# cyh-0/CAVP

Hardware: AMD Instinct MI355X
Metric: frames/sec end-to-end CAVP fwd+bwd, B=32 224x224 (higher is better)
Workload: dtype bf16; 1 GPU; C1' (config_avss_binary shape): CAVP ResNet-50 OS16 + VGGish, training step = forward_train (batch-stat BN, 32 images + 64 audio clips per GPU) + cross-entropy + full backward, 224x224 RGB + 96x64 mel, num_classes=2, random-init (synthetic) weights; global_batch=32, per_gpu_batch=32, parallelism=dp1, ranks=1, launch=hipGraph replay, deterministic=False

## Files before the change

### cavp_amd/_lib.py

```python
from __future__ import annotations

import ctypes as C
import os

import torch

HERE = os.path.dirname(os.path.abspath(__file__))
LIB_PATH = os.path.join(HERE, "libcavp_hip.so")

F32, BF16, I64 = 0, 1, 2
ACT_NONE, ACT_RELU, ACT_LEAKY, ACT_GELU = 0, 1, 2, 3
ABI_VERSION = 16
ERR_BAD_ARG, ERR_UNSUPPORTED, ERR_ALIGN, ERR_WORKSPACE, ERR_LAUNCH = -1, -2, -3, -4, -5
WGRAD_GROUP_MAX = 16


class CavpError(RuntimeError):
    pass


class ConvDesc(C.Structure):
    _fields_ = [(n, C.c_int32) for n in (
        "dtype", "N", "H", "W", "Cin", "ldx", "Cout", "ldy", "KH", "KW", "stride", "pad", "dil", "ldr", "act",
        "splitk", "tile", "up", "Ho", "Wo", "stride_w", "dw_oihw", "dw_overwrite", "res_rows", "aux_mode", "ld_aux")]
# ... 67 lines not shown
    "cavp_grad_accumulate": (_i32, [_vp, _i32, _i32, _vp, _vp, _vp, _vp]),
    "cavp_accum_advance": (_i32, [_vp, _vp, _vp, _vp]),
    "cavp_optimizer_schedule_gated": (_i32, [_vp, _vp, _vp]),
    "cavp_optimizer_step_dev_gated": (_i32, [_vp, _i32, _i32, C.c_float, C.c_float, _vp, _vp, _vp]),
    "cavp_grad_guard_partials_gated": (_i32, [_vp, _i32, _i32, _vp, _vp, _vp]),
    "cavp_grad_guard_finish_gated": (_i32, [_vp, _i32, _i32, _vp, _vp, _vp, _vp]),
    "cavp_optimizer_schedule_guarded_gated": (_i32, [_vp, _vp, _vp, _vp, _vp, _vp]),
    "cavp_optimizer_step_guarded_gated": (_i32, [_vp, _i32, _i32, C.c_float, C.c_float, _vp, _vp, _vp, _vp]),
    "cavp_rollback_range_bytes": (C.c_int64, []),
    "cavp_rollback_state_bytes": (C.c_int64, []),
    "cavp_rollback_blocks": (C.c_int64, [C.c_int64, C.c_int64]),
    "cavp_rollback_save": (_i32, [_vp, _i32, _i32, _vp, _vp]),
    "cavp_rollback_restore": (_i32, [_vp, _i32, _i32, _vp, _vp, _vp]),
    "cavp_mel_frontend": (_i32, [_vp, _i32, _i32, _vp, _vp, _vp, _i32, _i32, _i32, _i32, C.c_float, C.c_float, C.c_float, _vp]),
    "cavp_unpack_weight_grad": (_i32, [_vp, _vp, _i32, _i32, _i32, _i32, _i32, _vp]),
    "cavp_conv3x3_smallcin_wgrad": (_i32, [_i32, _vp, _vp, _vp, _i32, _i32, _i32, _i32, _i32, _i32, _vp, C.c_size_t, _vp]),
    "cavp_conv3x3_smallcin_wgrad_workspace_bytes": (C.c_size_t, [_i32, _i32, _i32, _i32, _i32, _i32, _i32]),
    "cavp_colstats": (_i32, [_i32, _vp, _vp, _i64, _i32, _i32, _vp, _vp, _vp]),
    "cavp_scale_f32": (_i32, [_vp, _f32, _vp, _i32, _vp]),
    "cavp_bn_finalize": (_i32, [_vp, _vp, _vp, _i64, _vp, _vp, _f32, _f32, _vp, _vp, _vp, _vp, _vp, _vp, _i32, _vp]),
    "cavp_conv2d_bnbwd_layout": (_i32, [_vp, _vp, _vp]),
    "cavp_conv2d_nhwc_bnbwd": (_i32, [_vp, _vp, _vp, _vp, _vp, _vp, _vp, _sz, _vp]),
    "cavp_bn_bwd_sum_tiles": (_i32, [_vp, _i32, _i32, _vp, _vp, _vp]),
    "cavp_scale_shift_act": (_i32, [_i32, _vp, _vp, _vp, _vp, _vp, _i64, _i32, _i32, _i32, _i32, _i32, _vp]),
    "cavp_bn_act_bwd_reduce": (_i32, [_i32, _vp, _vp, _vp, _vp, _vp, _i64, _i32, _i32, _i32, _i32, _i32, _vp, _vp, _vp, _vp,
                                      _vp]),
    "cavp_bn_act_bwd_apply": (_i32, [_i32, _vp, _vp, _vp, _vp, _vp, _vp, _vp, _vp, _i64, _i32, _i32, _i32, _i32, _i32,
                                     _vp, _i32, _vp, _i32, _vp, _vp, _vp]),
    "cavp_bn_act_bwd_apply_acc": (_i32, [_i32, _vp, _vp, _vp, _vp, _vp, _vp, _vp, _vp, _i64, _i32, _i32, _i32, _i32, _i32,
                                         _vp, _i32, _vp, _i32, _vp, _vp, _vp, _vp, _vp]),
    "cavp_bn_tiles_scale_shift_act": (_i32, [_i32, _vp, _vp, _i32, _i32, _vp, _vp, _f32, _f32, _vp, _vp, _vp, _vp, _vp, _vp, _vp, _vp,
                                             _i64, _i32, _i32, _i32, _i32, _i32, _vp]),
    "cavp_bn_tiles_bwd_apply": (_i32, [_i32, _vp, _vp, _vp, _vp, _vp, _vp, _i32, _vp, _vp, _i64, _i32, _i32, _i32, _vp, _i32, _vp]),
    "cavp_act_bwd": (_i32, [_i32, _vp, _vp, _vp, _i64, _i32, _i32, _i32, _i32, _i32, _vp]),
    "cavp_add": (_i32, [_i32, _vp, _vp, _vp, _i64, _vp]),
    "cavp_colsum": (_i32, [_i32, _vp, _i64, _i32, _i32, _vp, _vp]),
    "cavp_colsum_groups": (_i32, [_i32, _vp, _i32, _i32, _i32, _i32, _vp, _vp]),
    "cavp_col_tile_stats": (_i32, [_i32, _vp, _i64, _i32, _i32, _vp, _vp]),
    "cavp_layernorm_bwd": (_i32, [_i32, _vp, _vp, _vp, _vp, _vp, _vp, _i32, _i32, _i32, _i32, _i32, _f32, _vp]),
    "cavp_layernorm_bwd_add": (_i32, [_i32, _vp, _vp, _vp, _vp, _i32, _vp, _vp, _vp, _i32, _vp, _vp, _i32, _i32, _i32, _i32, _i32, _f32,
                                      _vp]),
    "cavp_attn_gate_bwd": (_i32, [_i32, _vp, _vp, _vp, _vp, _vp, _vp, _vp, _vp, _vp, _i32, _i32, _i32, _i32, _f32, _i32, _vp]),
    "cavp_maxpool_bwd_nhwc": (_i32, [_i32, _vp, _vp, _vp, _i32, _i32, _i32, _i32, _i32, _i32, _i32, _vp]),
    "cavp_bilinear_bwd_nhwc": (_i32, [_i32, _vp, _vp, _i32, _i32, _i32, _i32, _i32, _i32, _i32, _i32, _i32, _vp]),
    "cavp_bilinear_bwd_nchw_to_nhwc": (_i32, [_i32, _vp, _vp, _i32, _i32, _i32, _i32, _i32, _i32, _i32, _i32, _i32, _vp]),
    "cavp_bcast_add_nhwc": (_i32, [_i32, _vp, _vp, _f32, _i32, _i32, _i32, _i32, _vp]),
    "cavp_ce_loss_nchw": (_i32, [_vp, _vp, _i32, _i32, _i32, _i64, _i32, _f32, _vp, _vp, _vp, _vp]),
    "cavp_upsample_ce_head": (_i32, [_i32, _vp, _vp, _i32, _i32, _i32, _i32, _i32, _i32, _i32, _i32, _i32, _i32, _f32, _vp, _vp,
                              _vp, _vp, _vp]),
    "cavp_label_nearest": (_i32, [_vp, _vp, _i32, _i32, _i32, _i32, _i32, _vp]),
    "cavp_gather_l2norm": (_i32, [_vp, _i64, _i64, _i64, _vp, _i64, _i64, _i64, _vp, _vp, _vp, _i32, _i32, _i32, _i32, _i32, _f32, _vp,
                                  _vp, _vp]),
    "cavp_infonce_rows": (_i32, [_vp, _vp, _vp, _i32, _i32, _i32, _f32, _vp, _vp, _vp, _f32, _vp]),
    "cavp_symm_add": (_i32, [_vp, _vp, _i32, _f32, _vp, _vp]),
    "cavp_l2norm_bwd_scatter": (_i32, [_vp, _vp, _vp, _vp, _vp, _vp, _i32, _i32, _i32, _i32, _vp, _i64, _i64, _i64, _vp, _i64, _i64,
                                       _i64, _vp]),
    "cavp_contrast_sample_work_bytes": (_sz, [_i32]),
    "cavp_contrast_sample": (_i32, [_vp, _vp, _i64, _i32, _i32, _i32, _i32, _vp, _vp, _vp, _vp, _vp, _vp, _vp]),
    "cavp_contrast_gather_nhwc": (_i32, [_i32, _vp, _i32, _i32, _i32, _i32, _vp, _vp, _vp, _i32, _i32, _i32, _i32, _f32, _vp, _vp, _vp]),
    "cavp_contrast_rows_bwd_add": (_i32, [_i32, _vp, _i32, _i32, _i32, _i32, _vp, _vp, _vp, _i32, _i32, _i32, _vp, _vp, _vp, _f32,
                                          _vp]),
    "cavp_sra_attention": (_i32, [_i32, _vp, _vp, _vp, _i32, _i32, _i32, _i32, _i32, _f32, _vp]),
    "cavp_dwconv3x3_nhwc": (_i32, [_i32, _vp, _vp, _vp, _vp, _i32, _i32, _i32, _i32, _i32, _vp]),
    "cavp_dwconv3x3_nhwc_aux": (_i32, [_i32, _vp, _vp, _vp, _vp, _vp, _i32, _i32, _i32, _i32, _i32, _vp]),
    "cavp_dwconv3x3_bwd_data_nhwc": (_i32, [_i32, _vp, _vp, _vp, _i32, _i32, _i32, _i32, _vp]),
    "cavp_pack_dwconv_weight": (_i32, [_vp, _vp, _i32, _vp]),
# ... 108 lines not shown
```

### cavp_amd/csrc/train_pointwise.hip

```cpp
#include <stdlib.h>

#include <algorithm>
#include <cmath>

#include "common.h"
#include "host_util.h"

namespace {

__device__ __forceinline__ float act_grad_from_out(float y, int act) {
  switch (act) {
    case CAVP_ACT_RELU: return y > 0.f ? 1.f : 0.f;
    case CAVP_ACT_LEAKY: return y > 0.f ? 1.f : 0.01f;
    default: return 1.f;
  }
}

inline int cdiv_h(long long a, long long b) { return (int)((a + b - 1) / b); }

struct ColArgs {
  const void* a;
  const void* b;
  const void* c;
  const float* mean;
// ... 1819 lines not shown
    return CAVP_ERR_BAD_ARG;
  if ((running_mean == nullptr) != (running_var == nullptr)) return CAVP_ERR_BAD_ARG;
  if (!dt_ok(dtype) || tiles > bn_fused_tiles_limit()) return CAVP_ERR_UNSUPPORTED;
  const int VE = dt_ve(dtype);
  if (C % VE || ldx % VE || ldy % VE || (residual && ldr % VE)) return CAVP_ERR_UNSUPPORTED;
  if (!al16(x) || !al16(y) || (residual && !al16(residual)) || ((uintptr_t)tile_stats & 7)) return CAVP_ERR_UNSUPPORTED;
  const int gy = cdiv_h(C, BNF_SW);
  const int rpb = bn_fused_rows_per_block(rows, gy, 256 / (BNF_SW / VE));
  const dim3 grid(cdiv_h(rows, rpb), gy);
  cavp_dispatch_dtype(dtype, [&](auto t) { using T = decltype(t);
    bn_tiles_scale_shift_act_kernel<T><<<grid, 256, 0, (hipStream_t)stream>>>((const T*)x, tile_stats, tiles, rows_per_tile, rows, gamma, beta, eps, momentum, running_mean, running_var, scale, shift, mean, rstd, (const T*)residual, (T*)y, C, rpb, ldx, ldr, ldy, act); });
  CHECK_LAUNCH();
}

extern "C" int cavp_bn_tiles_bwd_apply(int32_t dtype, const void* dy, const void* z, const float* mean, const float* rstd,
                                       const float* gamma, const float* partials, int32_t tiles, float* sum_g, float* sum_gz,
                                       int64_t rows, int32_t C, int32_t ld_dy, int32_t ld_z, void* dz, int32_t ld_dz, void* stream) {
  if (!dy || !z || !mean || !rstd || !gamma || !partials || !sum_g || !sum_gz || !dz || tiles <= 0 || rows <= 0 || C <= 0 || ld_dy < C ||
      ld_z < C || ld_dz < C)
    return CAVP_ERR_BAD_ARG;
  if (!dt_ok(dtype) || tiles > bn_fused_tiles_limit()) return CAVP_ERR_UNSUPPORTED;
  const int VE = dt_ve(dtype);
  if (C % VE || ld_dy % VE || ld_z % VE || ld_dz % VE) return CAVP_ERR_UNSUPPORTED;
  if (!al16(dy) || !al16(z) || !al16(dz) || ((uintptr_t)partials & 7)) return CAVP_ERR_UNSUPPORTED;
  const float inv_m = (float)(1.0 / (double)rows);
  const int gy = cdiv_h(C, BNF_SW);
  const int rpb = bn_fused_rows_per_block(rows, gy, 256 / (BNF_SW / VE));
  const dim3 grid(cdiv_h(rows, rpb), gy);
  cavp_dispatch_dtype(dtype, [&](auto t) { using T = decltype(t);
    bn_tiles_bwd_apply_kernel<T><<<grid, 256, 0, (hipStream_t)stream>>>((const T*)dy, (const T*)z, mean, rstd, gamma, partials, tiles, inv_m, sum_g, sum_gz, (T*)dz, rows, C, rpb, ld_dy, ld_z, ld_dz); });
  CHECK_LAUNCH();
}

extern "C" int cavp_bn_act_bwd_reduce(int32_t dtype, const void* dy, const void* y, const void* z, const float* mean,
                                      const float* rstd, int64_t rows, int32_t C, int32_t ld_dy, int32_t ld_y,
                                      int32_t ld_z, int32_t act, float* sum_g, float* sum_gz, const float* fwd_scale,
                                      const float* fwd_shift, void* stream) {
  if (!dy || !z || !mean || !rstd || !sum_g || !sum_gz || rows <= 0 || C <= 0) return CAVP_ERR_BAD_ARG;
  if (!y && act != CAVP_ACT_NONE && (!fwd_scale || !fwd_shift)) return CAVP_ERR_BAD_ARG;
  if (!dt_ok(dtype) || rows > 0x7fffffff) return CAVP_ERR_UNSUPPORTED;
  const int VE = dt_ve(dtype);
  if (C % VE || ld_dy % VE || (y && ld_y % VE) || ld_z % VE) return CAVP_ERR_UNSUPPORTED;
  if (!al16(dy) || (y && !al16(y)) || !al16(z)) return CAVP_ERR_ALIGN;
  ColArgs a{};
  a.a = dy; a.b = y; a.c = z; a.mean = mean; a.rstd = rstd; a.out0 = sum_g; a.out1 = sum_gz;
  a.fscale = fwd_scale; a.fshift = fwd_shift;
  a.rows = (int)rows; a.C = C; a.lda = ld_dy; a.ldb = ld_y; a.ldc = ld_z; a.act = act;
  return launch_col_reduce<1>(dtype, a, (hipStream_t)stream);
}

extern "C" int cavp_bn_act_bwd_apply_acc(int32_t dtype, const void* dy, const void* y, const void* z, const float* mean,
                                         const float* rstd, const float* gamma, const float* sum_g, const float* sum_gz,
                                         int64_t rows, int32_t C, int32_t ld_dy, int32_t ld_y, int32_t ld_z, int32_t act,
                                         void* dz, int32_t ld_dz, void* g_out, int32_t ld_g, const float* fwd_scale,
                                         const float* fwd_shift, float* dbeta_acc, float* dgamma_acc, void* stream);
extern "C" int cavp_bn_act_bwd_apply(int32_t dtype, const void* dy, const void* y, const void* z, const float* mean,
                                     const float* rstd, const float* gamma, const float* sum_g, const float* sum_gz,
                                     int64_t rows, int32_t C, int32_t ld_dy, int32_t ld_y, int32_t ld_z, int32_t act,
                                     void* dz, int32_t ld_dz, void* g_out, int32_t ld_g, const float* fwd_scale,
                                     const float* fwd_shift, void* stream) {
  return cavp_bn_act_bwd_apply_acc(dtype, dy, y, z, mean, rstd, gamma, sum_g, sum_gz, rows, C, ld_dy, ld_y, ld_z, act, dz, ld_dz, g_out,
                                   ld_g, fwd_scale, fwd_shift, nullptr, nullptr, stream);
}

extern "C" int cavp_bn_act_bwd_apply_acc(int32_t dtype, const void* dy, const void* y, const void* z, const float* mean,
                                         const float* rstd, const float* gamma, const float* sum_g, const float* sum_gz,
// ... 435 lines not shown
```

### cavp_amd/train.py

```python
from __future__ import annotations

import os
from typing import Callable, Dict, List, Optional, Tuple

import torch
import torch.nn as nn

from . import ops
from . import train_ops as T
from ._lib import ACT_GELU, ACT_LEAKY, ACT_NONE, ACT_RELU, CavpError
from ._lib import load as _lib_load


class V:
    __slots__ = ("t", "_g", "parent", "lo", "hi", "needs_grad", "tile_stats", "grad_mul", "g_premul", "dp_scale", "g_scaled",
                 "bnb", "bnb_claim", "bnb_part")

    def __init__(self, t: torch.Tensor, parent: Optional["V"] = None, lo: int = 0, hi: int = 0, needs_grad: bool = True):
        self.t, self._g, self.parent, self.lo, self.hi, self.needs_grad = t, None, parent, lo, hi, needs_grad
        self.tile_stats = None
        self.grad_mul, self.g_premul = None, False
        self.dp_scale, self.g_scaled = None, None
        self.bnb, self.bnb_claim, self.bnb_part = None, None, None

# ... 165 lines not shown
    torch.maximum(st["bad"], mism, out=st["bad"])
    st["host"].copy_(st["bad"], non_blocking=True)
    st["event"] = torch.cuda.Event()
    st["event"].record(torch.cuda.current_stream())
    st["last"] = shape_key
    return torch.where(mism > 0, torch.full_like(mism, float("nan")), torch.zeros_like(mism)).reshape(())


def gather_bn_moments(local: torch.Tensor) -> torch.Tensor:
    import torch.distributed as dist
    world = dist.get_world_size()
    if dist.get_backend() == "nccl":
        out = torch.empty((world,) + tuple(local.shape), dtype=local.dtype, device=local.device)
        dist.all_gather_into_tensor(out, local.contiguous())
        return out
    out = torch.zeros((world,) + tuple(local.shape), dtype=local.dtype, device=local.device)
    out[dist.get_rank()].copy_(local)
    dist.all_reduce(out)
    return out


_FUSE_TOKEN_PATH = True
_RANK1_ATTN = True
_SIDE_STREAM = True
_GROUP_WGRAD = True
_BRANCH_STREAM = True
_SIDE_PACKS = True
_FUSE_BN_BWD = True
_BN_COMBINE_IN_APPLY = True
_BN_COMBINE_FWD_TILES = 1
_BN_COMBINE_BWD_TILES = 196
_BN_BWD_READ_Y = False
_FUSE_AUDIO_STEM = True
_FUSE_STEM_POOL = True


def bump_counters(model, counters) -> None:
    if not counters:
        return
    if counters[0].device.type != "cuda" or any(c.dtype != torch.int64 or c.numel() != 1 for c in counters):
        torch._foreach_add_(counters, 1)
        return
    key = tuple(c.data_ptr() for c in counters)
    cache = model.__dict__.setdefault("_cavp_nbt_tables", {})
    tab = cache.get(key)
    if tab is None:
        if torch.cuda.is_current_stream_capturing():
            torch._foreach_add_(counters, 1)
            return
        tab = torch.tensor(key, dtype=torch.int64).to(counters[0].device)
        cache[key] = tab
    T.i64_add_table(tab, 1)


class TrainPass:
    def __init__(self, model, dtype: torch.dtype, arena: Optional[GradArena] = None):
        self.m = model
        self.dt = dtype
        self.arena = arena
        self.touched = set()
        self.tape: List[Callable[[], None]] = []
        self.grads: Dict[int, torch.Tensor] = {}
        self.P: Dict[str, _P] = {}
        self._pack_jobs = []
        self._nbt = []
        self.on_early_final: Optional[Callable[[], None]] = None
# ... 361 lines not shown
            T.bn_tiles_to_moments(ts, tiles, rpt, rows, local)
            gathered = gather_bn_moments(local)
            count = rows * world
            T.bn_finalize_tiles(gathered, world, rows, count, bn.weight.detach(), bn.bias.detach(), bn.eps, mom,
                                bn.running_mean if track else None, bn.running_var if track else None, scale, shift,
                                mean, rstd)
        if track and bn.num_batches_tracked is not None:
            self._nbt.append(bn.num_batches_tracked)
        am = None
        if pool is not None:
            if residual is not None or out is not None or z.t.dim() != 4:
                raise ValueError("bn_act(pool=...): plain NHWC BatchNorm + activation only")
            pk, ps, pp = pool
            n_, h_, w_, c_ = z.t.shape
            y = V(self.empty((n_, (h_ + 2 * pp - pk) // ps + 1, (w_ + 2 * pp - pk) // ps + 1, c_), z.t.dtype))
            am = torch.empty(y.t.shape, dtype=torch.uint8, device=self.dev)
            ops.maxpool(z.t, y.t, pk, ps, pp, argmax=am, scale=scale, shift=shift, act=act)
        else:
            y = out if out is not None else V(self.empty(z.t.shape, z.t.dtype))
            if fused_tiles is not None:
                T.scale_shift_act(z.t, scale, shift, y.t, act, residual=residual.t if residual is not None else None,
                                  bn_tiles=fused_tiles)
            else:
                T.scale_shift_act(z.t, scale, shift, y.t, act, residual=residual.t if residual is not None else None)

        self._use(residual)
        if _FUSE_BN_BWD and not sync and not frozen and act == ACT_RELU and y.parent is None and z.t.dim() == 4 and pool is None:
            y.bnb = dict(z=z.t, out=y.t if residual is not None else None, scale=scale, shift=shift, mean=mean, rstd=rstd, act=act)

        def bwd():
            dy = y.g
            if dy is None:
                return
            if pool is not None:
                dpool = dy if dy.is_contiguous() else self._dense_copy(dy)
                dy = self.empty(z.t.shape, z.t.dtype)
                T.maxpool_bwd(am, dpool, dy, *pool)
            direct = (not sync and id(bn.weight) not in self.grads and id(bn.bias) not in self.grads)
            if y.bnb_part is not None:
                part, tiles = y.bnb_part
                dz = self.empty(z.t.shape, z.t.dtype)
                sums = (self.grad_buffer(bn.bias), self.grad_buffer(bn.weight)) if direct else self.zeros_f32(2, c)
                if _BN_COMBINE_IN_APPLY and tiles <= _BN_COMBINE_BWD_TILES:
                    T.bn_act_bwd_apply(dy, None, z.t, mean, rstd, bn.weight.detach(), sums[0], sums[1], ACT_NONE, dz,
                                       tile_partials=(part, tiles))
                else:
                    T.bn_bwd_sum_tiles(part, tiles, sums[0], sums[1])
                    T.bn_act_bwd_apply(dy, None, z.t, mean, rstd, bn.weight.detach(), sums[0], sums[1], ACT_NONE, dz)
                z.set_g(dz)
                if residual is not None and residual.needs_grad:
                    self.acc_add(residual, dy)
                if not direct:
                    self.add_grad(bn.bias, sums[0].clone())
                    self.add_grad(bn.weight, sums[1].clone())
                return
            if direct:
                sums = (self.grad_buffer(bn.bias), self.grad_buffer(bn.weight))
            else:
                sums = self.zeros_f32(2, c)
            yb = y.t if ((residual is not None or _BN_BWD_READ_Y) and pool is None) else None
            T.bn_act_bwd_reduce(dy, yb, z.t, mean, rstd, act, sums[0], sums[1], fwd_scale=scale, fwd_shift=shift)
            local = sums
            if sync and not frozen:
                import torch.distributed as dist
                local = sums.clone()
                dist.all_reduce(sums)
                sums = sums * (float(rows) / float(count))
            if frozen:
                sums = self.zeros_f32(2, c)
            dz = self.empty(z.t.shape, z.t.dtype)
            g_out = self.empty(z.t.shape, z.t.dtype) if (residual is not None and residual.needs_grad) else None
            T.bn_act_bwd_apply(dy, yb, z.t, mean, rstd, bn.weight.detach(), sums[0], sums[1], act, dz, g_out=g_out,
                               fwd_scale=scale, fwd_shift=shift)
            z.set_g(dz)
            if g_out is not None:
                self.acc_add(residual, g_out)
            if not direct:
                self.add_grad(bn.bias, local[0].clone())
                self.add_grad(bn.weight, local[1].clone())
        self.tape.append(bwd)
        return y

    def gelu(self, x: V) -> V:
        self._use(x)
        y = V(self.empty(x.t.shape, x.t.dtype))
        T.scale_shift_act(x.t, None, None, y.t, ACT_GELU)

        def bwd():
            if y.g is None:
                return
            def f(o, r):
                if r is None:
                    T.act_bwd(y.g, x.t, o, ACT_GELU)
                else:
                    tmp = self.empty(x.t.shape, x.t.dtype)
                    T.act_bwd(y.g, x.t, tmp, ACT_GELU)
                    T.add(r, tmp, o)
            self.acc(x, f)
        self.tape.append(bwd)
        return y

    def maxpool(self, x: V, k: int, stride: int, pad: int) -> V:
        self._use(x)
        n, h, w, c = x.t.shape
        y = V(self.empty((n, (h + 2 * pad - k) // stride + 1, (w + 2 * pad - k) // stride + 1, c)))
        am = torch.empty(y.t.shape, dtype=torch.uint8, device=self.dev)
# ... 852 lines not shown
```

### cavp_amd/train_ops.py

```python
from __future__ import annotations

import ctypes as C
from typing import Optional, Tuple

import torch

from . import _lib, ops
from ._lib import ConvDesc
from .ops import _need_gpu, _nhwc, _ptr, _stream, dtype_code


def _rows(t: torch.Tensor) -> Tuple[int, int, int]:
    c = t.shape[-1]
    if t.dim() == 1:
        return 1, c, c
    if t.stride(-1) != 1 and c > 1:
        raise _lib.CavpError("last dim must be contiguous")
    lead = [(s, st) for s, st in zip(t.shape[:-1], t.stride()[:-1]) if s > 1]
    rows = 1
    for s, _ in lead:
        rows *= s
    if not lead:
        return 1, c, c
    ld = lead[-1][1]
# ... 281 lines not shown
    ldr = 0
    if residual is not None:
        _, _, ldr = _rows(residual)
    _need_gpu(x, y, scale, shift, residual)
    if (rows, c) != (r2, c2) or y.dtype != x.dtype:
        raise _lib.CavpError("scale_shift_act: shape mismatch")
    if bn_tiles is not None:
        ts, tiles, rpt, gamma, beta, eps, momentum, rmean, rvar, mean, rstd = bn_tiles
        _need_gpu(ts, gamma, beta, mean, rstd)
        if scale is None or shift is None or gamma.numel() != c:
            raise _lib.CavpError("scale_shift_act(bn_tiles=...): scale / shift outputs of C elements required")
        st = _lib.load().cavp_bn_tiles_scale_shift_act(dtype_code(x.dtype), _ptr(x), _ptr(ts), tiles, rpt, _ptr(gamma), _ptr(beta),
                                                       C.c_float(eps), C.c_float(momentum), _ptr(rmean), _ptr(rvar), _ptr(scale),
                                                       _ptr(shift), _ptr(mean), _ptr(rstd), _ptr(residual), _ptr(y), rows, c, ldx,
                                                       ldr, ldy, act, _s())
        if st != _lib.ERR_UNSUPPORTED:
            _check(st, "cavp_bn_tiles_scale_shift_act")
            return y
        _bn_finalize_tiles(ts, tiles, rpt, rows, gamma, beta, eps, momentum, rmean, rvar, scale, shift, mean, rstd)
    _check(_lib.load().cavp_scale_shift_act(dtype_code(x.dtype), _ptr(x), _ptr(scale), _ptr(shift), _ptr(residual), _ptr(y),
                                            rows, c, ldx, ldr, ldy, act, _s()), "cavp_scale_shift_act")
    return y


def _bn_bwd_sum_tiles(partials, tiles: int, sum_g, sum_gz) -> None:
    _need_gpu(partials, sum_g, sum_gz)
    _check(_lib.load().cavp_bn_bwd_sum_tiles(_ptr(partials), tiles, sum_g.numel(), _ptr(sum_g), _ptr(sum_gz), _s()), "cavp_bn_bwd_sum_tiles")


def bn_bwd_sum_tiles(partials, tiles: int, sum_g, sum_gz) -> None:
    _bn_bwd_sum_tiles(partials, tiles, sum_g, sum_gz)


def bn_act_bwd_reduce(dy, y, z, mean, rstd, act: int, sum_g, sum_gz, fwd_scale=None, fwd_shift=None) -> None:
    rows, c, ld_dy = _rows(dy)
    ld_y = _rows(y)[2] if y is not None else 0
    _, _, ld_z = _rows(z)
    _need_gpu(dy, y, z, mean, rstd, sum_g, sum_gz, fwd_scale, fwd_shift)
    _check(_lib.load().cavp_bn_act_bwd_reduce(dtype_code(dy.dtype), _ptr(dy), _ptr(y), _ptr(z), _ptr(mean), _ptr(rstd), rows,
                                              c, ld_dy, ld_y, ld_z, act, _ptr(sum_g), _ptr(sum_gz), _ptr(fwd_scale),
                                              _ptr(fwd_shift), _s()),
           "cavp_bn_act_bwd_reduce")


def bn_act_bwd_apply(dy, y, z, mean, rstd, gamma, sum_g, sum_gz, act: int, dz, g_out=None, fwd_scale=None,
                     fwd_shift=None, acc=None, tile_partials=None) -> torch.Tensor:
    rows, c, ld_dy = _rows(dy)
    ld_y = _rows(y)[2] if y is not None else 0
    _, _, ld_z = _rows(z)
    _, _, ld_dz = _rows(dz)
    ld_g = _rows(g_out)[2] if g_out is not None else 0
    _need_gpu(dy, y, z, dz, g_out)
    if tile_partials is not None:
        part, tiles = tile_partials
        _need_gpu(part, mean, rstd, gamma, sum_g, sum_gz)
        if y is not None or g_out is not None or acc is not None or act != 0 or sum_g.numel() != c or sum_gz.numel() != c:
            raise _lib.CavpError("bn_act_bwd_apply(tile_partials=...): masked gradient only (y None, ACT_NONE, no g_out, no acc)")
        st = _lib.load().cavp_bn_tiles_bwd_apply(dtype_code(dy.dtype), _ptr(dy), _ptr(z), _ptr(mean), _ptr(rstd), _ptr(gamma),
                                                 _ptr(part), tiles, _ptr(sum_g), _ptr(sum_gz), rows, c, ld_dy, ld_z, _ptr(dz), ld_dz,
                                                 _s())
        if st != _lib.ERR_UNSUPPORTED:
            _check(st, "cavp_bn_tiles_bwd_apply")
            return dz
        _bn_bwd_sum_tiles(part, tiles, sum_g, sum_gz)
    _check(_lib.load().cavp_bn_act_bwd_apply_acc(dtype_code(dy.dtype), _ptr(dy), _ptr(y), _ptr(z), _ptr(mean), _ptr(rstd),
                                                 _ptr(gamma), _ptr(sum_g), _ptr(sum_gz), rows, c, ld_dy, ld_y, ld_z, act, _ptr(dz),
                                                 ld_dz, _ptr(g_out), ld_g, _ptr(fwd_scale), _ptr(fwd_shift),
                                                 _ptr(acc[0]) if acc is not None else None, _ptr(acc[1]) if acc is not None else None, _s()),
           "cavp_bn_act_bwd_apply")
    return dz


def act_bwd(dy, ref, dx, act: int) -> torch.Tensor:
    rows, c, ld_dy = _rows(dy)
    _, _, ld_ref = _rows(ref)
    _, _, ld_dx = _rows(dx)
    _need_gpu(dy, ref, dx)
    _check(_lib.load().cavp_act_bwd(dtype_code(dy.dtype), _ptr(dy), _ptr(ref), _ptr(dx), rows, c, ld_dy, ld_ref, ld_dx, act,
                                    _s()), "cavp_act_bwd")
# ... 275 lines not shown
```

### include/cavp_hip.h

```cpp
#ifndef CAVP_HIP_H_
#define CAVP_HIP_H_

#include <stddef.h>
#include <stdint.h>

#ifdef __cplusplus
extern "C" {
#endif

#define CAVP_ABI_VERSION 16

typedef enum { CAVP_F32 = 0, CAVP_BF16 = 1, CAVP_I64 = 2  } cavp_dtype_t;
typedef enum { CAVP_ACT_NONE = 0, CAVP_ACT_RELU = 1, CAVP_ACT_LEAKY = 2, CAVP_ACT_GELU = 3 } cavp_act_t;
typedef enum {
  CAVP_OK = 0,
  CAVP_ERR_BAD_ARG = -1,
  CAVP_ERR_UNSUPPORTED = -2,
  CAVP_ERR_ALIGN = -3,
  CAVP_ERR_WORKSPACE = -4,
  CAVP_ERR_LAUNCH = -5
} cavp_status_t;

int cavp_abi_version(void);

// ... 125 lines not shown
                                int32_t Cin, int32_t H, int32_t W, int32_t Cout, int32_t stride, void* workspace,
                                size_t workspace_bytes, void* stream);

int cavp_colstats(int32_t dtype, const void* x, const float* shift, int64_t rows, int32_t C, int32_t ldx, float* sum,
                  float* sumsq, void* stream);
int cavp_scale_f32(const float* in, float alpha, float* out, int32_t n, void* stream);
int cavp_bn_finalize(const float* sum, const float* sumsq, const float* stat_shift, int64_t count, const float* gamma,
                     const float* beta, float eps, float momentum, float* running_mean, float* running_var, float* scale, float* shift,
                     float* mean, float* rstd, int32_t C, void* stream);
int cavp_bn_finalize_tiles(const float* tile_stats, int32_t tiles, int32_t rows_per_tile, int64_t count,
                           const float* gamma, const float* beta, float eps, float momentum, float* running_mean,
                           float* running_var, float* scale, float* shift, float* mean, float* rstd, int32_t C,
                           void* stream);
int cavp_bn_tiles_to_moments(const float* tile_stats, int32_t tiles, int32_t rows_per_tile, int64_t count, float* moments,
                             int32_t C, void* stream);
int cavp_scale_shift_act(int32_t dtype, const void* x, const float* scale, const float* shift, const void* residual,
                         void* y, int64_t rows, int32_t C, int32_t ldx, int32_t ldr, int32_t ldy, int32_t act,
                         void* stream);
int cavp_bn_act_bwd_reduce(int32_t dtype, const void* dy, const void* y, const void* z, const float* mean,
                           const float* rstd, int64_t rows, int32_t C, int32_t ld_dy, int32_t ld_y, int32_t ld_z,
                           int32_t act, float* sum_g, float* sum_gz, const float* fwd_scale, const float* fwd_shift,
                           void* stream);
int cavp_bn_act_bwd_apply(int32_t dtype, const void* dy, const void* y, const void* z, const float* mean,
                          const float* rstd, const float* gamma, const float* sum_g, const float* sum_gz, int64_t rows,
                          int32_t C, int32_t ld_dy, int32_t ld_y, int32_t ld_z, int32_t act, void* dz, int32_t ld_dz,
                          void* g_out, int32_t ld_g, const float* fwd_scale, const float* fwd_shift, void* stream);
int cavp_bn_tiles_scale_shift_act(int32_t dtype, const void* x, const float* tile_stats, int32_t tiles, int32_t rows_per_tile,
                                  const float* gamma, const float* beta, float eps, float momentum, float* running_mean,
                                  float* running_var, float* scale, float* shift, float* mean, float* rstd, const void* residual,
                                  void* y, int64_t rows, int32_t C, int32_t ldx, int32_t ldr, int32_t ldy, int32_t act, void* stream);
int cavp_bn_tiles_bwd_apply(int32_t dtype, const void* dy, const void* z, const float* mean, const float* rstd, const float* gamma,
                            const float* partials, int32_t tiles, float* sum_g, float* sum_gz, int64_t rows, int32_t C,
                            int32_t ld_dy, int32_t ld_z, void* dz, int32_t ld_dz, void* stream);
int cavp_act_bwd(int32_t dtype, const void* dy, const void* ref, void* dx, int64_t rows, int32_t C, int32_t ld_dy,
                 int32_t ld_ref, int32_t ld_dx, int32_t act, void* stream);
int cavp_add(int32_t dtype, const void* a, const void* b, void* out, int64_t n, void* stream);
int cavp_colsum(int32_t dtype, const void* x, int64_t rows, int32_t C, int32_t ldx, float* out, void* stream);
int cavp_col_tile_stats(int32_t dtype, const void* x, int64_t rows, int32_t C, int32_t ldx, float* tile_stats, void* stream);
int cavp_colsum_groups(int32_t dtype, const void* x, int32_t groups, int32_t rows_per_group, int32_t C, int32_t ldx, float* out,
                       void* stream);
int cavp_layernorm_bwd(int32_t dtype, const void* dy, const void* x, const float* gamma, void* dx, float* dgamma,
                       float* dbeta, int32_t rows, int32_t C, int32_t ld_dy, int32_t ld_x, int32_t ld_dx, float eps,
                       void* stream);
int cavp_layernorm_bwd_add(int32_t dtype, const void* dy, const void* x, const float* gamma, const void* dx_add, int32_t ld_add,
                           void* dx, void* dx_scaled, const float* row_scale, int32_t rows_per_group, float* dgamma,
                           float* dbeta, int32_t rows, int32_t C, int32_t ld_dy, int32_t ld_x, int32_t ld_dx, float eps,
                           void* stream);
int cavp_attn1_supported(int32_t C, int32_t heads);
int cavp_attn1_prepare(int32_t dtype, const float* wq, const float* wp, const void* k, const void* v, float* U, float* P, int32_t B,
                       int32_t C, int32_t heads, float scale, void* stream);
int cavp_attn1_fwd(int32_t dtype, const void* x, const float* U, const float* P, const float* bp, void* out, float* attn, int32_t B,
                   int32_t xb, int32_t T, int32_t C, int32_t heads, void* stream);
size_t cavp_attn1_bwd_workspace_bytes(int32_t B, int32_t xb, int32_t T, int32_t C, int32_t heads);
int cavp_attn1_bwd(int32_t dtype, const void* dout, const void* x, const float* U, const float* P, void* dx, float* dU, float* dP,
                   float* dbp, void* workspace, size_t workspace_bytes, int32_t B, int32_t xb, int32_t T, int32_t C, int32_t heads,
                   void* stream);
int cavp_attn1_finish(int32_t dtype, const float* wq, const float* wp, const void* k, const void* v, const float* dU, const float* dP,
                      float* dwq, float* dwp, float* dk, float* dv, int32_t B, int32_t C, int32_t heads, float scale, void* stream);
int cavp_attn_gate_bwd(int32_t dtype, const void* dout, const void* q, const void* k, const void* v, const float* attn,
                       const float* dattn, void* dq, float* dk, float* dv, int32_t B, int32_t T, int32_t heads,
                       int32_t hd, float scale, int32_t q_batch, void* stream);
int cavp_maxpool_bwd_nhwc(int32_t dtype, const uint8_t* argmax, const void* dy, void* dx, int32_t N, int32_t H, int32_t W,
                          int32_t C, int32_t k, int32_t stride, int32_t pad, void* stream);
int cavp_bilinear_bwd_nhwc(int32_t dtype, const void* dy, void* dx, int32_t N, int32_t Hi, int32_t Wi, int32_t C,
                           int32_t ld_dx, int32_t Ho, int32_t Wo, int32_t ld_dy, int32_t align_corners, void* stream);
int cavp_bilinear_bwd_nchw_to_nhwc(int32_t dtype, const float* dy_nchw, void* dx, int32_t N, int32_t n_valid,
// ... 337 lines not shown
```

Baseline: 2431 frames/s.

## Fuse stem maxpool backward into BN backward reduce and apply kernels

Adds two HIP kernels that recompute the maxpool backward gradient from the argmax and pooled gradient while doing the batch-norm backward reduction and apply for the stem. This avoids materialising the full-resolution pre-pool gradient tensor and the separate maxpool_bwd launch. The cost is that the scatter-gather is done twice (once in reduce, once in apply). It also adds a partials workspace allocation and a fallback path when the shapes are unsupported.

After: 2438 frames/s, median of 6. About the same (+0.3%).

```diff
diff --git a/cavp_amd/_lib.py b/cavp_amd/_lib.py
--- a/cavp_amd/_lib.py
+++ b/cavp_amd/_lib.py
@@ -123,6 +123,10 @@
     "cavp_bn_tiles_scale_shift_act": (_i32, [_i32, _vp, _vp, _i32, _i32, _vp, _vp, _f32, _f32, _vp, _vp, _vp, _vp, _vp, _vp, _vp, _vp,
                                              _i64, _i32, _i32, _i32, _i32, _i32, _vp]),
     "cavp_bn_tiles_bwd_apply": (_i32, [_i32, _vp, _vp, _vp, _vp, _vp, _vp, _i32, _vp, _vp, _i64, _i32, _i32, _i32, _vp, _i32, _vp]),
+    "cavp_bn_pool_bwd_reduce": (_i32, [_i32, _vp, _vp, _vp, _vp, _vp, _vp, _vp, _i32, _i32, _i32, _i32, _i32, _i32, _i32, _i32, _vp, _i32,
+                                       _vp, _vp, _vp]),
+    "cavp_bn_pool_bwd_apply": (_i32, [_i32, _vp, _vp, _vp, _vp, _vp, _vp, _vp, _vp, _vp, _vp, _i32, _i32, _i32, _i32, _i32, _i32, _i32,
+                                      _i32, _vp, _vp]),
     "cavp_act_bwd": (_i32, [_i32, _vp, _vp, _vp, _i64, _i32, _i32, _i32, _i32, _i32, _vp]),
     "cavp_add": (_i32, [_i32, _vp, _vp, _vp, _i64, _vp]),
     "cavp_colsum": (_i32, [_i32, _vp, _i64, _i32, _i32, _vp, _vp]),
diff --git a/cavp_amd/csrc/train_pointwise.hip b/cavp_amd/csrc/train_pointwise.hip
--- a/cavp_amd/csrc/train_pointwise.hip
+++ b/cavp_amd/csrc/train_pointwise.hip
@@ -1875,6 +1875,277 @@
   CHECK_LAUNCH();
 }
 
+template <typename T>
+__device__ __forceinline__ void round_to_storage(float* v) {
+  if constexpr (!std::is_same<T, float>::value) {
+    constexpr int VE = VecT<T>::VE;
+    uint4 t;
+    t.x = pack2bf(v[0], v[1]); t.y = pack2bf(v[2], v[3]); t.z = pack2bf(v[4], v[5]); t.w = pack2bf(v[6], v[7]);
+    static_assert(VE == 8, "bf16 vectors hold 8 elements");
+    VecT<T>::unpack(t, v);
+  }
+}
+
+template <typename T>
+__device__ __forceinline__ void pool_s2_gather(const unsigned char* __restrict__ argmax, const T* __restrict__ dpool, int n, int hi, int wi,
+                                               int cv, int C, int k, int pad, int Ho, int Wo, float* acc) {
+  constexpr int VE = VecT<T>::VE;
+#pragma unroll
+  for (int e = 0; e < VE; ++e) acc[e] = 0.f;
+  const int ho_lo = hi + pad - k + 1 <= 0 ? 0 : (hi + pad - k + 2) >> 1;
+  const int ho_hi = min((hi + pad) >> 1, Ho - 1);
+  const int wo_lo = wi + pad - k + 1 <= 0 ? 0 : (wi + pad - k + 2) >> 1;
+  const int wo_hi = min((wi + pad) >> 1, Wo - 1);
+  uint4 gr[2][2];
+  uint2 ar[2][2];
+  bool ok[2][2];
+#pragma unroll
+  for (int i = 0; i < 2; ++i)
+#pragma unroll
+    for (int j = 0; j < 2; ++j) {
+      const int ho = ho_lo + i, wo = wo_lo + j;
+      ok[i][j] = ho <= ho_hi && wo <= wo_hi;
+      gr[i][j] = make_uint4(0u, 0u, 0u, 0u);
+      ar[i][j] = make_uint2(0u, 0u);
+      if (ok[i][j]) {
+        const size_t o = ((size_t)(n * Ho + ho) * Wo + wo) * C + cv * VE;
+        if constexpr (VE == 8) ar[i][j] = *(const uint2*)(argmax + o);
+        else ar[i][j].x = *(const unsigned*)(argmax + o);
+        gr[i][j] = VecT<T>::load_raw(dpool + o);
+      }
+    }
+#pragma unroll
+  for (int i = 0; i < 2; ++i)
+#pragma unroll
+    for (int j = 0; j < 2; ++j) {
+      if (!ok[i][j]) continue;
+      const unsigned code = (unsigned)((hi - ((ho_lo + i) * 2 - pad)) * k + (wi - ((wo_lo + j) * 2 - pad)));
+      float g[VE];
+      VecT<T>::unpack(gr[i][j], g);
+#pragma unroll
+      for (int e = 0; e < VE; ++e) {
+        const unsigned am = ((e < 4 ? ar[i][j].x : ar[i][j].y) >> (8 * (e & 3))) & 255u;
+        acc[e] += am == code ? g[e] : 0.f;
+      }
+    }
+  round_to_storage<T>(acc);
+}
+
+template <typename T, int CG>
+__global__ __launch_bounds__(256) void bn_pool_bwd_reduce_kernel(const unsigned char* __restrict__ argmax, const T* __restrict__ dpool,
+                                                                 const T* __restrict__ z, const float* __restrict__ mean,
+                                                                 const float* __restrict__ rstd, const float* __restrict__ fscale,
+                                                                 const float* __restrict__ fshift, float* __restrict__ part, int rows, int H,
+                                                                 int W, int C, int k, int pad, int Ho, int Wo, int rows_per_block, int act,
+                                                                 unsigned w_mul, unsigned w_sh, unsigned h_mul, unsigned h_sh) {
+  constexpr int VE = VecT<T>::VE;
+  constexpr int RL = 256 / CG;
+  __shared__ float red[2][RL][CG * VE + 1];
+  const int cg = threadIdx.x % CG, rl = threadIdx.x / CG;
+  const int cv = blockIdx.y * CG + cg, c0 = cv * VE;
+  const bool col_ok = c0 < C;
+  float s0[VE], s1[VE], mu[VE], rs[VE], fs[VE], fh[VE];
+#pragma unroll
+  for (int e = 0; e < VE; ++e) { s0[e] = s1[e] = 0.f; mu[e] = 0.f; rs[e] = 1.f; fs[e] = 1.f; fh[e] = 0.f; }
+  if (col_ok) {
+#pragma unroll
+    for (int e = 0; e < VE; ++e) { mu[e] = mean[c0 + e]; rs[e] = rstd[c0 + e]; }
+    if (act != CAVP_ACT_NONE) {
+#pragma unroll
+      for (int e = 0; e < VE; ++e) { fs[e] = fscale[c0 + e]; fh[e] = fshift[c0 + e]; }
+    }
+    const float slope = act_grad_from_out(-1.f, act);
+    const int r_begin = blockIdx.x * rows_per_block, r_end = min(r_begin + rows_per_block, rows);
+#pragma unroll 2
+    for (int r = r_begin + rl; r < r_end; r += RL) {
+      float a[VE], zz[VE];
+      VecT<T>::load(z + (size_t)r * C + c0, zz);
+      const int row = fast_div(r, w_mul, w_sh), wi = r - row * W;
+      const int n = fast_div(row, h_mul, h_sh), hi = row - n * H;
+      pool_s2_gather<T>(argmax, dpool, n, hi, wi, cv, C, k, pad, Ho, Wo, a);
+#pragma unroll
+      for (int e = 0; e < VE; ++e) {
+        const float yv = zz[e] * fs[e] + fh[e];
+        const float g = a[e] * (yv > 0.f ? 1.f : slope);
+        s0[e] += g;
+        s1[e] += g * (zz[e] - mu[e]) * rs[e];
+      }
+    }
+  }
+#pragma unroll
+  for (int e = 0; e < VE; ++e) {
+    red[0][rl][cg * VE + e] = s0[e];
+    red[1][rl][cg * VE + e] = s1[e];
+  }
+  __syncthreads();
+  for (int i = threadIdx.x; i < 2 * CG * VE; i += 256) {
+    const int st = i / (CG * VE), ch = i - st * (CG * VE);
+    const int c = blockIdx.y * CG * VE + ch;
+    if (c >= C) continue;
+    float s = 0.f;
+#pragma unroll
+    for (int q = 0; q < RL; ++q) s += red[st][q][ch];
+    part[((size_t)st * gridDim.x + blockIdx.x) * C + c] = s;
+  }
+}
+
+constexpr int PBA_ROWS = 8;
+__device__ __forceinline__ int pool_s2_lo(int i, int k, int pad) { return i + pad - k + 1 <= 0 ? 0 : (i + pad - k + 2) >> 1; }
+template <typename T>
+__global__ __launch_bounds__(256) void bn_pool_bwd_apply_kernel(const unsigned char* __restrict__ argmax, const T* __restrict__ dpool,
+                                                                const T* __restrict__ z, const float* __restrict__ mean,
+                                                                const float* __restrict__ rstd, const float* __restrict__ gamma,
+                                                                const float* __restrict__ sum_g, const float* __restrict__ sum_gz,
+                                                                float inv_m, const float* __restrict__ fscale,
+                                                                const float* __restrict__ fshift, T* __restrict__ dz, int NP, int HP, int H,
+                                                                int W, int C, int k, int pad, int Ho, int Wo, int act, int cv_shift) {
+  constexpr int VE = VecT<T>::VE;
+  const int CV = C / VE;
+  const int t = blockIdx.x * 256 + threadIdx.x;
+  if (t >= W * CV) return;
+  const int wi = cv_shift >= 0 ? t >> cv_shift : t / CV;
+  const int cv = t - wi * CV, c = cv * VE;
+  float ca[VE], cb[VE], cc[VE], mu[VE], fs[VE], fh[VE];
+  {
+    float rs[VE], gm[VE], sg[VE], sgz[VE];
+#pragma unroll
+    for (int q = 0; q < VE; q += 4) {
+      VecT<float>::load(rstd + c + q, rs + q); VecT<float>::load(gamma + c + q, gm + q); VecT<float>::load(sum_g + c + q, sg + q);
+      VecT<float>::load(sum_gz + c + q, sgz + q); VecT<float>::load(mean + c + q, mu + q);
+    }
+#pragma unroll
+    for (int e = 0; e < VE; ++e) { bn_bwd_coeffs(gm[e], rs[e], sg[e], sgz[e], inv_m, ca[e], cb[e], cc[e]); fs[e] = 1.f; fh[e] = 0.f; }
+    if (act != CAVP_ACT_NONE) {
+#pragma unroll
+      for (int q = 0; q < VE; q += 4) { VecT<float>::load(fscale + c + q, fs + q); VecT<float>::load(fshift + c + q, fh + q); }
+    }
+  }
+  const float slope = act_grad_from_out(-1.f, act);
+  const int wo_lo = pool_s2_lo(wi, k, pad), wo_hi = min((wi + pad) >> 1, Wo - 1);
+  const int p0 = blockIdx.y * (PBA_ROWS / 2), p1 = min(p0 + PBA_ROWS / 2, NP);
+  for (int pr = p0; pr < p1; ++pr) {
+    const int n = pr / HP, hi = (pr - n * HP) * 2;
+    const bool two = hi + 1 < H;
+    const size_t off = (((size_t)n * H + hi) * W + wi) * C + c, pitch = (size_t)W * C;
+    uint4 zr[2];
+    zr[0] = VecT<T>::load_raw(z + off);
+    zr[1] = two ? VecT<T>::load_raw(z + off + pitch) : make_uint4(0u, 0u, 0u, 0u);
+    const int hb = pool_s2_lo(hi, k, pad), ho_top = min((hi + (two ? 1 : 0) + pad) >> 1, Ho - 1);
+    uint4 gr[2][2];
+    uint2 ar[2][2];
+    bool ok[2][2];
+#pragma unroll
+    for (int i = 0; i < 2; ++i)
+#pragma unroll
+      for (int j = 0; j < 2; ++j) {
+        const int ho = hb + i, wo = wo_lo + j;
+        ok[i][j] = ho <= ho_top && wo <= wo_hi;
+        gr[i][j] = make_uint4(0u, 0u, 0u, 0u);
+        ar[i][j] = make_uint2(0u, 0u);
+        if (ok[i][j]) {
+          const size_t o = ((size_t)(n * Ho + ho) * Wo + wo) * C + c;
+          if constexpr (VE == 8) ar[i][j] = *(const uint2*)(argmax + o);
+          else ar[i][j].x = *(const unsigned*)(argmax + o);
+          gr[i][j] = VecT<T>::load_raw(dpool + o);
+        }
+      }
+#pragma unroll
+    for (int q = 0; q < 2; ++q) {
+      if (q == 1 && !two) break;
+      const int hq = hi + q, lo_q = pool_s2_lo(hq, k, pad), hi_q = min((hq + pad) >> 1, Ho - 1);
+      float a[VE], zz[VE], o[VE];
+#pragma unroll
+      for (int e = 0; e < VE; ++e) a[e] = 0.f;
+#pragma unroll
+      for (int i = 0; i < 2; ++i)
+#pragma unroll
+        for (int j = 0; j < 2; ++j) {
+          const int ho = hb + i;
+          if (!ok[i][j] || ho < lo_q || ho > hi_q) continue;
+          const unsigned code = (unsigned)((hq - (ho * 2 - pad)) * k + (wi - ((wo_lo + j) * 2 - pad)));
+          float g[VE];
+          VecT<T>::unpack(gr[i][j], g);
+#pragma unroll
+          for (int e = 0; e < VE; ++e) {
+            const unsigned am = ((e < 4 ? ar[i][j].x : ar[i][j].y) >> (8 * (e & 3))) & 255u;
+            a[e] += am == code ? g[e] : 0.f;
+          }
+        }
+      round_to_storage<T>(a);
+      VecT<T>::unpack(zr[q], zz);
+#pragma unroll
+      for (int e = 0; e < VE; ++e) {
+        const float yv = zz[e] * fs[e] + fh[e];
+        const float g = a[e] * (yv > 0.f ? 1.f : slope);
+        o[e] = bn_bwd_dz(ca[e], g, cb[e], zz[e], mu[e], cc[e]);
+      }
+      VecT<T>::store(dz + off + q * pitch, o);
+    }
+  }
+}
+
+inline int bn_pool_bwd_check(int32_t dtype, const void* argmax, const void* dpool, const void* z, int32_t N, int32_t H, int32_t W, int32_t C,
+                             int32_t k, int32_t stride, int32_t pad, int32_t act) {
+  if (!argmax || !dpool || !z || N <= 0 || H <= 0 || W <= 0 || C <= 0 || k <= 0 || stride <= 0 || pad < 0) return CAVP_ERR_BAD_ARG;
+  if (!dt_ok(dtype) || stride != 2 || (k != 2 && k != 3) || pad > 1 || H + 2 * pad < k || W + 2 * pad < k) return CAVP_ERR_UNSUPPORTED;
+  if (act != CAVP_ACT_NONE && act != CAVP_ACT_RELU && act != CAVP_ACT_LEAKY) return CAVP_ERR_UNSUPPORTED;
+  if (C % dt_ve(dtype) || (long long)N * ((H + 1) / 2) > 65535ll * (PBA_ROWS / 2) || (long long)W * C > 0x7fffffffll) return CAVP_ERR_UNSUPPORTED;
+  if (((uintptr_t)argmax & 7) || !al16(dpool) || !al16(z)) return CAVP_ERR_ALIGN;
+  return CAVP_OK;
+}
+
+extern "C" int cavp_bn_pool_bwd_reduce(int32_t dtype, const uint8_t* argmax, const void* dpool, const void* z, const float* mean,
+                                       const float* rstd, const float* fwd_scale, const float* fwd_shift, int32_t N, int32_t H,
+                                       int32_t W, int32_t C, int32_t k, int32_t stride, int32_t pad, int32_t act, float* partials,
+                                       int32_t max_tiles, float* sum_g, float* sum_gz, void* stream) {
+  if (!mean || !rstd || !partials || max_tiles <= 0 || !sum_g || !sum_gz) return CAVP_ERR_BAD_ARG;
+  if (act != CAVP_ACT_NONE && (!fwd_scale || !fwd_shift)) return CAVP_ERR_BAD_ARG;
+  const int st = bn_pool_bwd_check(dtype, argmax, dpool, z, N, H, W, C, k, stride, pad, act);
+  if (st != CAVP_OK) return st;
+  const int VE = dt_ve(dtype);
+  const long long rows = (long long)N * H * W;
+  if (rows > 0x7fffffffll) return CAVP_ERR_UNSUPPORTED;
+  const int CG = C <= 8 * VE ? 8 : 16;
+  const int gy = cdiv_h(C, CG * VE);
+  int gx = std::max(1, 768 / gy);
+  int rpb = std::max(cdiv_h(rows, gx), 64);
+  rpb = (rpb + 31) / 32 * 32;
+  gx = cdiv_h(rows, rpb);
+  if (gx > max_tiles) return CAVP_ERR_WORKSPACE;
+  const int Ho = (H + 2 * pad - k) / 2 + 1, Wo = (W + 2 * pad - k) / 2 + 1;
+  unsigned wm, ws, hm, hs;
+  fast_div_prepare(W, &wm, &ws);
+  fast_div_prepare(H, &hm, &hs);
+  hipStream_t s = (hipStream_t)stream;
+  cavp_dispatch_dtype(dtype, [&](auto t) { using T = decltype(t);
+    if (CG == 8) bn_pool_bwd_reduce_kernel<T, 8><<<dim3(gx, gy), 256, 0, s>>>(argmax, (const T*)dpool, (const T*)z, mean, rstd, fwd_scale, fwd_shift, partials, (int)rows, H, W, C, k, pad, Ho, Wo, rpb, act, wm, ws, hm, hs);
+    else bn_pool_bwd_reduce_kernel<T, 16><<<dim3(gx, gy), 256, 0, s>>>(argmax, (const T*)dpool, (const T*)z, mean, rstd, fwd_scale, fwd_shift, partials, (int)rows, H, W, C, k, pad, Ho, Wo, rpb, act, wm, ws, hm, hs); });
+  if (launch_status() != CAVP_OK) return CAVP_ERR_LAUNCH;
+  return cavp_det_finish(partials, gx, C, sum_g, sum_gz, s) == hipSuccess ? CAVP_OK : CAVP_ERR_LAUNCH;
+}
+
+extern "C" int cavp_bn_pool_bwd_apply(int32_t dtype, const uint8_t* argmax, const void* dpool, const void* z, const float* mean,
+                                      const float* rstd, const float* gamma, const float* sum_g, const float* sum_gz,
+                                      const float* fwd_scale, const float* fwd_shift, int32_t N, int32_t H, int32_t W, int32_t C,
+                                      int32_t k, int32_t stride, int32_t pad, int32_t act, void* dz, void* stream) {
+  if (!mean || !rstd || !gamma || !sum_g || !sum_gz || !dz) return CAVP_ERR_BAD_ARG;
+  if (act != CAVP_ACT_NONE && (!fwd_scale || !fwd_shift)) return CAVP_ERR_BAD_ARG;
+  const int st = bn_pool_bwd_check(dtype, argmax, dpool, z, N, H, W, C, k, stride, pad, act);
+  if (st != CAVP_OK) return st;
+  if (!al16(dz) || !al16(mean) || !al16(rstd) || !al16(gamma) || !al16(sum_g) || !al16(sum_gz) || (fwd_scale && (!al16(fwd_scale) || !al16(fwd_shift))))
+    return CAVP_ERR_ALIGN;
+  const int VE = dt_ve(dtype), NH = N * H, CV = C / VE;
+  const int Ho = (H + 2 * pad - k) / 2 + 1, Wo = (W + 2 * pad - k) / 2 + 1;
+  const float inv_m = (float)(1.0 / ((double)NH * W));
+  int sh = -1;
+  if ((CV & (CV - 1)) == 0) { sh = 0; while ((1 << sh) < CV) ++sh; }
+  const int HP = (H + 1) / 2, NP = N * HP;
+  const dim3 grid((W * CV + 255) / 256, cdiv_h(NP, PBA_ROWS / 2));
+  cavp_dispatch_dtype(dtype, [&](auto t) { using T = decltype(t);
+    bn_pool_bwd_apply_kernel<T><<<grid, 256, 0, (hipStream_t)stream>>>(argmax, (const T*)dpool, (const T*)z, mean, rstd, gamma, sum_g, sum_gz, inv_m, fwd_scale, fwd_shift, (T*)dz, NP, HP, H, W, C, k, pad, Ho, Wo, act, sh); });
+  CHECK_LAUNCH();
+}
+
 extern "C" int cavp_bn_act_bwd_reduce(int32_t dtype, const void* dy, const void* y, const void* z, const float* mean,
                                       const float* rstd, int64_t rows, int32_t C, int32_t ld_dy, int32_t ld_y,
                                       int32_t ld_z, int32_t act, float* sum_g, float* sum_gz, const float* fwd_scale,
diff --git a/cavp_amd/train.py b/cavp_amd/train.py
--- a/cavp_amd/train.py
+++ b/cavp_amd/train.py
@@ -221,6 +221,7 @@
 _BN_COMBINE_BWD_TILES = 196
 _BN_BWD_READ_Y = False
 _FUSE_AUDIO_STEM = True
+_FUSE_STEM_POOL_BWD = True
 _FUSE_STEM_POOL = True
 
 
@@ -648,10 +649,14 @@
             dy = y.g
             if dy is None:
                 return
+            pool_bwd = None
             if pool is not None:
                 dpool = dy if dy.is_contiguous() else self._dense_copy(dy)
-                dy = self.empty(z.t.shape, z.t.dtype)
-                T.maxpool_bwd(am, dpool, dy, *pool)
+                if _FUSE_STEM_POOL_BWD:
+                    pool_bwd, dy = (am, dpool) + tuple(pool), None
+                else:
+                    dy = self.empty(z.t.shape, z.t.dtype)
+                    T.maxpool_bwd(am, dpool, dy, *pool)
             direct = (not sync and id(bn.weight) not in self.grads and id(bn.bias) not in self.grads)
             if y.bnb_part is not None:
                 part, tiles = y.bnb_part
@@ -675,7 +680,10 @@
             else:
                 sums = self.zeros_f32(2, c)
             yb = y.t if ((residual is not None or _BN_BWD_READ_Y) and pool is None) else None
-            T.bn_act_bwd_reduce(dy, yb, z.t, mean, rstd, act, sums[0], sums[1], fwd_scale=scale, fwd_shift=shift)
+            if pool_bwd is not None:
+                dy = T.bn_act_bwd_reduce(None, None, z.t, mean, rstd, act, sums[0], sums[1], fwd_scale=scale, fwd_shift=shift, pool=pool_bwd)
+            else:
+                T.bn_act_bwd_reduce(dy, yb, z.t, mean, rstd, act, sums[0], sums[1], fwd_scale=scale, fwd_shift=shift)
             local = sums
             if sync and not frozen:
                 import torch.distributed as dist
@@ -687,7 +695,7 @@
             dz = self.empty(z.t.shape, z.t.dtype)
             g_out = self.empty(z.t.shape, z.t.dtype) if (residual is not None and residual.needs_grad) else None
             T.bn_act_bwd_apply(dy, yb, z.t, mean, rstd, bn.weight.detach(), sums[0], sums[1], act, dz, g_out=g_out,
-                               fwd_scale=scale, fwd_shift=shift)
+                               fwd_scale=scale, fwd_shift=shift, pool=pool_bwd)
             z.set_g(dz)
             if g_out is not None:
                 self.acc_add(residual, g_out)
diff --git a/cavp_amd/train_ops.py b/cavp_amd/train_ops.py
--- a/cavp_amd/train_ops.py
+++ b/cavp_amd/train_ops.py
@@ -337,7 +337,36 @@
     _bn_bwd_sum_tiles(partials, tiles, sum_g, sum_gz)
 
 
-def bn_act_bwd_reduce(dy, y, z, mean, rstd, act: int, sum_g, sum_gz, fwd_scale=None, fwd_shift=None) -> None:
+_POOL_BWD_MAX_TILES = 768
+
+
+def _pool_bwd_args(pool, z, what: str):
+    argmax, dpool, k, stride, pad = pool
+    _need_gpu(argmax, dpool, z)
+    if z.dim() != 4 or not z.is_contiguous() or not dpool.is_contiguous() or dpool.dtype != z.dtype:
+        raise _lib.CavpError(f"{what}(pool=...): dense NHWC z and pooled gradient of one dtype required")
+    if argmax.dtype != torch.uint8 or argmax.shape != dpool.shape or not argmax.is_contiguous():
+        raise _lib.CavpError(f"{what}(pool=...): dense uint8 argmax of the pooled gradient's shape required")
+    n, h, w, c = z.shape
+    if tuple(dpool.shape) != (n, (h + 2 * pad - k) // stride + 1, (w + 2 * pad - k) // stride + 1, c):
+        raise _lib.CavpError(f"{what}(pool=...): the pooled gradient does not have the pool's output shape")
+    return argmax, dpool, k, stride, pad, n, h, w, c
+
+
+def bn_act_bwd_reduce(dy, y, z, mean, rstd, act: int, sum_g, sum_gz, fwd_scale=None, fwd_shift=None, pool=None):
+    if pool is not None:
+        if dy is not None or y is not None:
+            raise _lib.CavpError("bn_act_bwd_reduce(pool=...): dy and y must be None")
+        argmax, dpool, k, stride, pad, n, h, w, c = _pool_bwd_args(pool, z, "bn_act_bwd_reduce")
+        _need_gpu(mean, rstd, sum_g, sum_gz, fwd_scale, fwd_shift)
+        part = torch.empty((2, _POOL_BWD_MAX_TILES, c), dtype=torch.float32, device=z.device)
+        st = _lib.load().cavp_bn_pool_bwd_reduce(dtype_code(z.dtype), _ptr(argmax), _ptr(dpool), _ptr(z), _ptr(mean), _ptr(rstd),
+                                                 _ptr(fwd_scale), _ptr(fwd_shift), n, h, w, c, k, stride, pad, act, _ptr(part),
+                                                 _POOL_BWD_MAX_TILES, _ptr(sum_g), _ptr(sum_gz), _s())
+        if st != _lib.ERR_UNSUPPORTED:
+            _check(st, "cavp_bn_pool_bwd_reduce")
+            return None
+        dy = maxpool_bwd(argmax, dpool, torch.empty_like(z), k, stride, pad)
     rows, c, ld_dy = _rows(dy)
     ld_y = _rows(y)[2] if y is not None else 0
     _, _, ld_z = _rows(z)
@@ -346,10 +375,25 @@
                                               c, ld_dy, ld_y, ld_z, act, _ptr(sum_g), _ptr(sum_gz), _ptr(fwd_scale),
                                               _ptr(fwd_shift), _s()),
            "cavp_bn_act_bwd_reduce")
+    return dy if pool is not None else None
 
 
 def bn_act_bwd_apply(dy, y, z, mean, rstd, gamma, sum_g, sum_gz, act: int, dz, g_out=None, fwd_scale=None,
-                     fwd_shift=None, acc=None, tile_partials=None) -> torch.Tensor:
+                     fwd_shift=None, acc=None, tile_partials=None, pool=None) -> torch.Tensor:
+    if pool is not None and dy is None:
+        if y is not None or g_out is not None or acc is not None or tile_partials is not None:
+            raise _lib.CavpError("bn_act_bwd_apply(pool=...): y None, no g_out, no acc, no tile_partials")
+        argmax, dpool, k, stride, pad, n, h, w, c = _pool_bwd_args(pool, z, "bn_act_bwd_apply")
+        _need_gpu(mean, rstd, gamma, sum_g, sum_gz, fwd_scale, fwd_shift, dz)
+        if dz.shape != z.shape or dz.dtype != z.dtype or not dz.is_contiguous():
+            raise _lib.CavpError("bn_act_bwd_apply(pool=...): dense dz of z's shape and dtype required")
+        st = _lib.load().cavp_bn_pool_bwd_apply(dtype_code(z.dtype), _ptr(argmax), _ptr(dpool), _ptr(z), _ptr(mean), _ptr(rstd),
+                                                _ptr(gamma), _ptr(sum_g), _ptr(sum_gz), _ptr(fwd_scale), _ptr(fwd_shift), n, h, w, c,
+                                                k, stride, pad, act, _ptr(dz), _s())
+        if st != _lib.ERR_UNSUPPORTED:
+            _check(st, "cavp_bn_pool_bwd_apply")
+            return dz
+        dy = maxpool_bwd(argmax, dpool, torch.empty_like(z), k, stride, pad)
     rows, c, ld_dy = _rows(dy)
     ld_y = _rows(y)[2] if y is not None else 0
     _, _, ld_z = _rows(z)
diff --git a/include/cavp_hip.h b/include/cavp_hip.h
--- a/include/cavp_hip.h
+++ b/include/cavp_hip.h
@@ -181,6 +181,14 @@
 int cavp_bn_tiles_bwd_apply(int32_t dtype, const void* dy, const void* z, const float* mean, const float* rstd, const float* gamma,
                             const float* partials, int32_t tiles, float* sum_g, float* sum_gz, int64_t rows, int32_t C,
                             int32_t ld_dy, int32_t ld_z, void* dz, int32_t ld_dz, void* stream);
+int cavp_bn_pool_bwd_reduce(int32_t dtype, const uint8_t* argmax, const void* dpool, const void* z, const float* mean, const float* rstd,
+                            const float* fwd_scale, const float* fwd_shift, int32_t N, int32_t H, int32_t W, int32_t C, int32_t k,
+                            int32_t stride, int32_t pad, int32_t act, float* partials, int32_t max_tiles, float* sum_g, float* sum_gz,
+                            void* stream);
+int cavp_bn_pool_bwd_apply(int32_t dtype, const uint8_t* argmax, const void* dpool, const void* z, const float* mean, const float* rstd,
+                           const float* gamma, const float* sum_g, const float* sum_gz, const float* fwd_scale, const float* fwd_shift,
+                           int32_t N, int32_t H, int32_t W, int32_t C, int32_t k, int32_t stride, int32_t pad, int32_t act, void* dz,
+                           void* stream);
 int cavp_act_bwd(int32_t dtype, const void* dy, const void* ref, void* dx, int64_t rows, int32_t C, int32_t ld_dy,
                  int32_t ld_ref, int32_t ld_dx, int32_t act, void* stream);
 int cavp_add(int32_t dtype, const void* a, const void* b, void* out, int64_t n, void* stream);
```
